# RobustFieldAutonomyLab/DRL_graph_exploration

Hardware: AMD Instinct MI355X
Metric: env-steps/sec (256 parallel envs, ~64-node graphs) (higher is better)
Workload: dtype f64; 1 GPU; configs[1]: 256 envs/GPU, 40x40 map (V=1600), 100 landmarks, belief update at ~59-node graphs (P=37.0 poses, L=22.2 landmarks, M=188 factors) from a device snapshot; envs_per_gpu=256, map_size=40, num_landmarks=100, parallelism=env-sharded x1

## Files before the change

drl_graph_exploration_amd/_lib.py:

```python
import ctypes as C
import os

from .config import DrlgxConfig

_HERE = os.path.dirname(os.path.abspath(__file__))
_PATH = os.environ.get("DRLGX_LIB_DEV", os.path.join(_HERE, "libdrlgx.so"))
_lib = None

N_TIMERS = 8


class DrlgxError(RuntimeError):
    pass


class CsrCache(C.Structure):
    _fields_ = [(n, C.c_void_p) for n in ("deg", "selfw", "ax", "ptr_dst", "end_dst", "ptr_src", "end_src", "nbr_dst", "nbr_src", "wn_dst",
                                          "wn_src")]
    NODE_WORDS = dict(deg=1, selfw=1, ax=8, ptr_dst=1, end_dst=1, ptr_src=1, end_src=1)
    EDGE_WORDS = dict(nbr_dst=1, nbr_src=1, wn_dst=1, wn_src=1)


def lib_path():
    return _PATH


SYMBOLS = [
    "drlgx_create", "drlgx_destroy", "drlgx_set_stream", "drlgx_synchronize", "drlgx_strerror", "drlgx_last_error",
    "drlgx_status_host", "drlgx_status_fetch_host", "drlgx_reset_host", "drlgx_step", "drlgx_utility", "drlgx_uncertainty_em", "drlgx_explored", "drlgx_metrics", "drlgx_cov_array",
    "drlgx_stage_reset_host", "drlgx_stage_set_prior_information_host", "drlgx_stage_set_prior_pose_host", "drlgx_stage_move", "drlgx_stage_measure", "drlgx_stage_add_measurements", "drlgx_stage_optimize",
    "drlgx_stage_update_map", "drlgx_set_planner_parameter", "drlgx_set_fixed_landmarks_host", "drlgx_fm2_update", "drlgx_fm2_update_steps", "drlgx_em_cost", "drlgx_em_cost_steps", "drlgx_set_dubins_leaf_scoring", "drlgx_em_plan_leaves", "drlgx_og_cost", "drlgx_slam_og_cost", "drlgx_set_sampler_parameter", "drlgx_set_sampler_obstacles", "drlgx_set_dubins_library_host", "drlgx_dubins_library", "drlgx_set_dubins_prefilter", "drlgx_em_plan", "drlgx_rrt_plan", "drlgx_step_plan", "drlgx_step_plans", "drlgx_step_plans_traced",
    "drlgx_line_plan", "drlgx_lookahead", "drlgx_lookahead_bounded", "drlgx_graph_capacity", "drlgx_graph", "drlgx_get_counts_host", "drlgx_counts",
    "drlgx_get_poses_host", "drlgx_get_landmarks_host", "drlgx_get_cov_traces_host", "drlgx_vm_shape",
    "drlgx_get_virtual_map_host", "drlgx_get_ground_truth_host", "drlgx_get_adjacency_host", "drlgx_get_factors_host",
    "drlgx_get_landmark_order_host", "drlgx_snapshot", "drlgx_restore", "drlgx_timing_enable",
    "drlgx_timing_read_host", "drlgx_debug_phase_clocks_host", "drlgx_debug_gemm_tile_rows", "drlgx_debug_map_form", "drlgx_debug_map_compact_ok", "drlgx_debug_disc_cells_bound", "drlgx_inc_stats_host", "drlgx_debug_panel_host", "drlgx_gcn_workspace_bytes", "drlgx_gcn_forward", "drlgx_gcn_forward_batched", "drlgx_gcn_backward",
    "drlgx_replay_collate", "drlgx_replay_collate_pair", "drlgx_dqn_targets", "drlgx_dqn_loss_grad", "drlgx_dqn_arena_bytes", "drlgx_dqn_arena_views", "drlgx_dqn_prepare", "drlgx_dqn_forward_backward", "drlgx_replay_cache_csr", "drlgx_gcn_collate_csr", "drlgx_gcn_forward_prebuilt", "drlgx_adam_step", "drlgx_adam_step_scaled", "drlgx_normalise_rewards",
    "drlgx_segment_softmax", "drlgx_segment_softmax_backward", "drlgx_mean_pool", "drlgx_mean_pool_backward",
    "drlgx_ggnn_workspace_bytes", "drlgx_ggnn_forward", "drlgx_ggnn_backward",
    "drlgx_greedy_plans",
    "drlgx_set_env_obstacles", "drlgx_obstacle_flags", "drlgx_follow_plans",
    "drlgx_unet_workspace_bytes", "drlgx_unet_forward", "drlgx_unet_backward", "drlgx_unet_topk", "drlgx_unet_augment_filter", "drlgx_unet_kept_nodes",
]


def lib():
    global _lib
    if _lib is not None:
        return _lib
    import torch
    if not os.path.exists(_PATH):
        raise DrlgxError(
            "libdrlgx.so not found at %s — build it with `python -c 'import __graft_entry__ as g; g.build()'` "
            "(hipcc --offload-arch=gfx950); there is no CPU fallback." % _PATH)
    L = C.CDLL(_PATH)
    vp, ip, dp = C.c_void_p, C.POINTER(C.c_int32), C.POINTER(C.c_double)
    L.drlgx_create.argtypes = [C.POINTER(DrlgxConfig), C.c_int, C.c_int, C.c_int, C.POINTER(vp)]
    L.drlgx_destroy.argtypes = [vp]
    L.drlgx_set_stream.argtypes = [vp, vp]
# ... 54 lines not shown
    L.drlgx_get_counts_host.argtypes = [vp, C.c_int, ip]
    L.drlgx_counts.argtypes = [vp, vp]
    L.drlgx_get_poses_host.argtypes = [vp, C.c_int, dp, dp]
    L.drlgx_get_landmarks_host.argtypes = [vp, C.c_int, ip, dp, dp]
    L.drlgx_get_cov_traces_host.argtypes = [vp, C.c_int, dp, dp]
    L.drlgx_vm_shape.argtypes = [vp, ip, ip]
    L.drlgx_get_virtual_map_host.argtypes = [vp, C.c_int, dp, dp, dp, C.POINTER(C.c_uint8)]
    L.drlgx_get_ground_truth_host.argtypes = [vp, C.c_int, dp, dp]
    L.drlgx_get_adjacency_host.argtypes = [vp, C.c_int, dp, dp]
    L.drlgx_get_factors_host.argtypes = [vp, C.c_int, ip, ip, dp, dp]
    L.drlgx_get_landmark_order_host.argtypes = [vp, ip]
    L.drlgx_snapshot.argtypes = [vp, C.c_int]
    L.drlgx_restore.argtypes = [vp, C.c_int]
    L.drlgx_timing_enable.argtypes = [vp, C.c_int]
    L.drlgx_timing_read_host.argtypes = [vp, dp, C.POINTER(C.c_int64)]
    L.drlgx_debug_phase_clocks_host.argtypes = [vp, C.c_int, C.POINTER(C.c_int64)]
    L.drlgx_debug_gemm_tile_rows.argtypes = [C.c_int, C.c_int, C.c_int, C.c_int]
    L.drlgx_debug_map_form.argtypes = [C.c_int]
    L.drlgx_debug_map_compact_ok.argtypes = [vp, C.c_int]
    L.drlgx_debug_disc_cells_bound.argtypes = [C.c_double]
    L.drlgx_inc_stats_host.argtypes = [vp, C.POINTER(C.c_int64), C.c_int]
    if os.environ.get("DRLGX_LIB_DEV") is None or hasattr(L, "drlgx_debug_panel_host"):
        L.drlgx_debug_panel_host.argtypes = [vp, C.c_int, ip, dp, C.c_size_t]
    L.drlgx_gcn_workspace_bytes.restype = C.c_size_t
    L.drlgx_gcn_workspace_bytes.argtypes = [C.c_int, C.c_int, C.c_int, C.c_int]
    L.drlgx_gcn_forward.argtypes = [vp] + [C.c_int] * 5 + [vp] * 12
    L.drlgx_gcn_backward.argtypes = [vp] + [C.c_int] * 5 + [vp] * 15
    L.drlgx_ggnn_workspace_bytes.restype = C.c_size_t
    L.drlgx_ggnn_workspace_bytes.argtypes = [C.c_int] * 5
    L.drlgx_ggnn_forward.argtypes = [vp] + [C.c_int] * 6 + [vp] * 13 + [C.c_int, vp, vp, C.c_int]
    L.drlgx_ggnn_backward.argtypes = [vp] + [C.c_int] * 6 + [vp] * 17
    L.drlgx_unet_workspace_bytes.restype = C.c_size_t
    L.drlgx_unet_workspace_bytes.argtypes = [C.c_int] * 6 + [C.c_double, C.c_int]
    L.drlgx_unet_forward.argtypes = [vp] + [C.c_int] * 5 + [C.c_double, C.c_int] + [vp] * 3 + [C.POINTER(vp)] + [vp] * 3 + [C.c_size_t, C.c_int, vp, vp,
                                                                                                                       C.c_int]
    L.drlgx_unet_backward.argtypes = [vp] + [C.c_int] * 5 + [C.c_double, C.c_int] + [vp] * 3 + [C.POINTER(vp), vp, vp, C.POINTER(vp), vp, C.c_size_t,
                                                                                                C.c_int, C.c_int]
    L.drlgx_unet_kept_nodes.argtypes = [vp] + [C.c_int] * 4 + [C.c_double, C.c_int, vp, C.c_size_t, C.c_int, C.c_int, C.c_int, vp, C.POINTER(C.c_int)]
    L.drlgx_unet_topk.argtypes = [vp, C.c_int, C.c_int, vp, vp, C.c_double, vp, vp, vp, vp]
    L.drlgx_unet_augment_filter.argtypes = [vp, C.c_int, C.c_int, vp, vp, C.c_int, vp, vp, C.c_int, vp, vp, vp, C.c_int64, vp, vp, vp]
    L.drlgx_replay_collate.argtypes = [vp, C.c_int, vp, vp, C.c_int, vp, C.c_int64, vp, vp, vp, C.c_int64, vp, vp, vp, vp, vp, vp]
    L.drlgx_replay_collate_pair.argtypes = [vp, C.c_int, vp, vp, C.c_int, vp, C.c_int64, vp, vp, vp, C.c_int64, vp, vp, vp, vp, vp, vp, vp]
    L.drlgx_gcn_forward_batched.argtypes = [vp] + [C.c_int] * 5 + [vp] * 12 + [C.c_int, vp, vp, C.c_int]
    L.drlgx_dqn_targets.argtypes = [vp, C.c_int, vp, vp, vp, C.c_double, C.c_int64, vp, vp]
    L.drlgx_dqn_loss_grad.argtypes = [vp, C.c_int, vp, vp, vp, C.c_double, vp, vp]
    i64 = C.c_int64
# ... 41 lines not shown
```

drl_graph_exploration_amd/csrc/drlgx_dev.h:

```cpp
#pragma once
#include <hip/hip_runtime.h>
#include <stdint.h>

#include "../../include/drlgx.h"
#include "map_carve.h"

#define DRLGX_MT_N 624
#define DRLGX_MT_STRIDE 626
#define DRLGX_CNT_STRIDE 8
#define DRLGX_RED_STRIDE 8
#define DRLGX_PRIOR_STRIDE 16

enum { C_P = 0, C_L = 1, C_M = 2, C_STEP = 3, C_ISAM = 4, C_NEWP = 5, C_NEWL = 6, C_FLAG = 7 };
enum { R_UTR = 0, R_KNOWN = 1, R_EXPL = 2, R_UDET = 3, R_UWTR = 4, R_DIST = 5, R_OBS = 6, R_LATCH = 7 };

struct DrlgxState {
  drlgx_config cfg;
  int n_envs, n_inst, n_roll;
  int P_max, L_max, M_max, LG, V, Vu, rows, cols, A_max;
  int win;
  int disc_cells;
  int count_explored;
  double lo_free, lo_occ, lo_min, lo_max, occ_thresh;
  int bbox_noop;
// ... 559 lines not shown
size_t drlgx_simlog_entry_bytes(const DrlgxState &S);
void drlgx_launch_presim(const DrlgxState &S, hipStream_t st, LaunchSel sel, const double *odom, int odom_stride, int n_measure, int a_end,
                         unsigned char *simlog, size_t simlog_roll, int simlog_act);
void drlgx_launch_sim(const DrlgxState &S, hipStream_t st, LaunchSel sel, const double *odom, int odom_stride,
                      int n_measure);
void drlgx_launch_sim_obs(const DrlgxState &S, hipStream_t st, LaunchSel sel, const double *odom, int odom_stride);
void drlgx_launch_slam(const DrlgxState &S, hipStream_t st, LaunchSel sel, int p_bound);
size_t drlgx_map_lds_bytes(const DrlgxState &S, int *chunk_out, int pcap = 0);
bool drlgx_step_fusable(const DrlgxState &S, int p_bound);
bool drlgx_step_arrow_fusable(const DrlgxState &S);
void drlgx_launch_step_arrow(const DrlgxState &S, hipStream_t st, LaunchSel sel, const double *odom, int odom_stride, int n_measure);
void drlgx_launch_step(const DrlgxState &S, hipStream_t st, LaunchSel sel, const double *odom, int odom_stride, int n_measure);
void drlgx_launch_step_loop(const DrlgxState &S, hipStream_t st, LaunchSel sel, const double *odom, int odom_stride, int n_measure, int a_end);
void drlgx_launch_step_arrow_loop(const DrlgxState &S, hipStream_t st, LaunchSel sel, const double *odom, int odom_stride, int n_measure, int a_end);
void drlgx_launch_map(const DrlgxState &S, hipStream_t st, LaunchSel sel, int rebuild);
bool drlgx_map_two_per_cu(const DrlgxState &S, int p_bound);
bool drlgx_map_compact_ok(const DrlgxState &S, int p_bound);
void drlgx_launch_copy(const DrlgxField *fields_dev, int n_fields, hipStream_t st, int n, const int32_t *src,
                       const int32_t *dst, int src_off, int dst_off, int skip_mask,
                       const int *cnt = nullptr,
                       const DrlgxState *panel = nullptr,
                       int only_cls = -1,
                       int panel_mode = 1);
void drlgx_launch_rebase(const DrlgxState &S, hipStream_t st, int base0, int n);
inline size_t drlgx_fetch_head_bytes(int n_envs) { return ((size_t)(n_envs + 1) * sizeof(int) + 15) & ~(size_t)15; }
void drlgx_launch_fetch_pack(const DrlgxState &S, hipStream_t st, const void *src, size_t bytes, void *out);
void drlgx_launch_fix_rollouts(const DrlgxState &S, hipStream_t st, int n_cand, const int32_t *cand_env, int roll0);
void drlgx_launch_rewards(const DrlgxState &S, hipStream_t st, int n_cand, const int32_t *cand_env, int roll0,
                          double *rewards);
void drlgx_launch_utility(const DrlgxState &S, hipStream_t st, const double *dist, double *out, int mode);
void drlgx_launch_fm2_prior(const DrlgxState &S, hipStream_t st, const int32_t *env_ids, int n_env, double *sig, size_t sig_stride,
                            int n_max);
size_t drlgx_fm2_scratch_doubles(const DrlgxState &S, int nm_max);
void drlgx_launch_fm2_check(const DrlgxState &S, hipStream_t st, int n_cand, const int32_t *cand_env, const double *actions,
                            const int32_t *n_actions, const uint8_t *core, int nm_max, int *flag);
void drlgx_launch_fm2_update(const DrlgxState &S, hipStream_t st, int c0, int nc, const int32_t *cand_env, const int32_t *env_slot,
                             const double *actions, const int32_t *n_actions, const uint8_t *core, const double *sig, size_t sig_stride,
                             double *scratch, size_t scratch_stride, int *iscratch, int nm_max, double *cov_out, int out_stride,
                             int32_t *n_out, double *lm_out = nullptr, int lm_stride = 0);
void drlgx_launch_fm2_prior_ordered(const DrlgxState &S, hipStream_t st, double *sig, size_t sig_stride, int n_max);
size_t drlgx_em_lds_bytes(const DrlgxState &S);
void drlgx_launch_em_cost(const DrlgxState &S, hipStream_t st, int nc, const int32_t *cand_env, const double *actions,
                          const int32_t *n_actions, const uint8_t *core, const double *distance, const double *cov, int cov_stride,
                          int algorithm, double *unc_out, double *cost_out, double *info_out);
size_t drlgx_og_lds_bytes(const DrlgxState &S);
void drlgx_launch_og_check(const DrlgxState &S, hipStream_t st, int n_cand, const int32_t *cand_env, const int32_t *n_actions, int *flag);
// ... 61 lines not shown
```

drl_graph_exploration_amd/csrc/drlgx_engine.cpp:

```cpp
#include <hip/hip_runtime.h>

#include <algorithm>
#include <chrono>
#include <cmath>
#include <cstdio>
#include <cstring>
#include <functional>
#include <string>
#include <unordered_map>
#include <cstdlib>
#include <vector>

#include "drlgx_dev.h"
#include "drlgx_fields.h"

#define HIPCHK(e, call)                                                                       \
  do {                                                                                        \
    hipError_t _r = (call);                                                                   \
    if (_r != hipSuccess) {                                                                   \
      (e)->last_error = std::string(#call) + ": " + hipGetErrorString(_r);                    \
      return DRLGX_E_HIP;                                                                     \
    }                                                                                         \
  } while (0)

struct TimedSpan {
  hipEvent_t a, b;
  int id;
};

struct drlgx_engine {
  DrlgxState S{};
  int device = 0;
  hipStream_t own_stream = nullptr, stream = nullptr;
  std::vector<void *> allocs;
  DrlgxState *state_dev = nullptr;
  unsigned char state_shadow[sizeof(DrlgxState)];
  std::vector<DrlgxField> fields;
  DrlgxField *fields_dev = nullptr;
  std::vector<int> lm_order;
  int32_t *stage_i32 = nullptr;
  uint32_t *stage_u32 = nullptr;
  double *stage_f64 = nullptr;
  uint8_t *stage_mask = nullptr;
  int *graph_gi = nullptr;
  int graph_gi_stride = 0;
  bool timing = false;
  std::vector<int> pbound;
  bool by_capacity = false;
  std::vector<std::vector<int>> snap_pbound;
  bool per_stage = false;
  std::vector<TimedSpan> spans;
  std::vector<hipEvent_t> free_events;
  double t_ms[DRLGX_N_TIMERS] = {0};
  int64_t t_n[DRLGX_N_TIMERS] = {0};
  std::string last_error;
  double *fixed_lm_dev = nullptr;
  unsigned char *simlog_dev = nullptr;
  bool la_presim = true;
  bool spin_sync = true;
  hipEvent_t sync_event = nullptr;
  unsigned char *fetch_dev = nullptr, *fetch_host = nullptr;
// ... 14 lines not shown
  int *tree_link = nullptr, *tree_leaf = nullptr, *tree_meta = nullptr;
  int32_t *tree_cand_env = nullptr, *tree_cand_n = nullptr;
  size_t tree_nodes_cap = 0, tree_sel_cap = 0, tree_cand_cap = 0;
  double sampler_max_nodes = 0.5, sampler_safe_distance = 0.0;
  int sampler_dubins = 0;
  int sampler_obstacles = 0;
  int env_obstacles = 0;
  double *follow_act = nullptr;
  int dubins_leaf_scoring = 0;
  uint8_t *tree_cand_core = nullptr;
  double *tree_cand_dist = nullptr;
  size_t tree_cand_steps_cap = 0, tree_cand_last = 0;
  bool tree_cand_last_steps = false;
  DrlgxDubins dubins = {};
  double *dub_end_x = nullptr, *dub_end_y = nullptr, *dub_v = nullptr, *dub_w = nullptr, *tree_pose = nullptr;
  int *dub_steps = nullptr;
  size_t dub_cap = 0, tree_pose_cap = 0;
  double dub_reach = 0.0;
  int dub_prefilter = 1;
  std::vector<double> dub_end_h, dub_v_h, dub_w_h;
  std::vector<int> dub_steps_h;
  int owed_slot = -1;
  bool restore_eager = false;
};

#define DRLGX_ENTER_OWING(e)                    \
  do {                                          \
    if (e) {                                    \
      (void)hipSetDevice((e)->device);          \
      state_sync(e);                            \
    }                                           \
  } while (0)
#define DRLGX_ENTER(e)                          \
  do {                                          \
    DRLGX_ENTER_OWING(e);                       \
    if (e) settle(e);                           \
  } while (0)

struct drlgx_engine;
static void state_sync(drlgx_engine *e);
static void settle(drlgx_engine *e);

namespace {

template <typename T>
int dev_alloc(drlgx_engine *e, T **out, size_t count) {
// ... 86 lines not shown
  }
  const int LG = std::max(cfg->num_landmarks, 1);
  if (drlgx_sim_launch_lds(DRLGX_SIM_RESET, LG) > kSimLdsLimit || drlgx_sim_launch_lds(DRLGX_SIM_STEP, LG) > kSimLdsLimit ||
      drlgx_sim_launch_lds(DRLGX_SIM_STAGE, LG) > kSimLdsLimit ||
      (n_rollouts > 0 && drlgx_sim_launch_lds(DRLGX_SIM_PRESIM, LG, 1) > kSimLdsLimit)) {
    g_create_error = "num_landmarks too large for the LDS of the simulator kernels (k_reset / k_sim_step / k_presim)";
    return DRLGX_E_INVALID;
  }
  return DRLGX_OK;
}

static bool env_flag(const char *name, bool dflt) {
  const char *v = getenv(name);
  if (!v) return dflt;
  return dflt ? v[0] != '0' : v[0] == '1';
}

static void read_env_switches(drlgx_engine *e) {
  e->by_capacity = env_flag("DRLGX_VARIANT_BY_CAPACITY", false);
  e->spin_sync = env_flag("DRLGX_SYNC_SPIN", true);
  e->la_presim = env_flag("DRLGX_LOOKAHEAD_PRESIM", true);
  e->la_loop = env_flag("DRLGX_LOOKAHEAD_LOOP", true);
  e->restore_eager = env_flag("DRLGX_RESTORE_EAGER", false);
}

static double p2l(double p) { return std::log(p / (1.0 - p)); }
static double l2p(double l) { return std::exp(l) / (1.0 + std::exp(l)); }

static int disc_cells_bound(double r) {
  const int n = 32;
  const double h = 0.5 / n, rr = r + h * 0.70710678118654752440 + 1e-9;
  const int k = (int)std::ceil(rr) + 1;
  int best = 0;
  for (int a = 0; a < n; ++a)
    for (int b = 0; b < n; ++b) {
      const double u = (a + 0.5) * h, v = (b + 0.5) * h;
      int cnt = 0;
      for (int i = -k; i <= k; ++i)
        for (int j = -k; j <= k; ++j)
          if ((i - u) * (i - u) + (j - v) * (j - v) <= rr * rr) ++cnt;
      best = std::max(best, cnt);
    }
  return best;
}

static int set_map_constants(drlgx_engine *e) {
// ... 192 lines not shown
    while (e->allocs.size() > n_before) {
      hipFree(e->allocs.back());
      e->allocs.pop_back();
    }
    S.jc = nullptr;
    S.jd = nullptr;
    S.jc_meta = nullptr;
    S.inc_stats = nullptr;
    e->last_error.clear();
    fprintf(stderr, "drlgx: covariance panels (%.1f GB) not allocated (budget %.1f GB): every belief update is a full solve\n", gb, max_gb);
  }
  return DRLGX_OK;
}

static int alloc_staging(drlgx_engine *e) {
  DrlgxState &S = e->S;
  const int n_envs = S.n_envs;
  TRY(dev_alloc(e, &S.status, 1));
  std::stable_sort(e->fields.begin(), e->fields.end(), [](const DrlgxField &a, const DrlgxField &b) {
    return (a.pad > 0 ? (size_t)a.pad : a.stride) > (b.pad > 0 ? (size_t)b.pad : b.stride);
  });
  TRY(dev_alloc(e, &e->fields_dev, e->fields.size()));
  HIPCHK(e, hipMemcpyAsync(e->fields_dev, e->fields.data(), e->fields.size() * sizeof(DrlgxField), hipMemcpyHostToDevice, e->stream));
  TRY(dev_alloc(e, &e->stage_i32, (size_t)n_envs));
  TRY(dev_alloc(e, &e->stage_u32, (size_t)n_envs));
  TRY(dev_alloc(e, &e->stage_f64, (size_t)n_envs * 3));
  TRY(dev_alloc(e, &e->stage_mask, (size_t)n_envs));
  e->graph_gi_stride = 4 * S.L_max + 8;
  TRY(dev_alloc(e, &e->graph_gi, (size_t)n_envs * e->graph_gi_stride));
  unsigned char *raw = nullptr;
  TRY(dev_alloc(e, &raw, sizeof(DrlgxState)));
  e->state_dev = reinterpret_cast<DrlgxState *>(raw);
  S.self_dev = e->state_dev;
  return DRLGX_OK;
}

static int build_engine(drlgx_engine *e) {
  DrlgxState &S = e->S;
  const drlgx_config *cfg = &S.cfg;
  if (cfg->max_snapshots < 0 || cfg->max_snapshots > 16) return DRLGX_E_INVALID;
  S.n_inst = 2 * S.n_envs + S.n_roll + cfg->max_snapshots * S.n_envs;
  e->pbound.assign(S.n_envs, cfg->max_poses);
  e->snap_pbound.assign(cfg->max_snapshots > 0 ? cfg->max_snapshots : 0, std::vector<int>(S.n_envs, cfg->max_poses));
  read_env_switches(e);
  hipDeviceProp_t prop;
  if (hipGetDeviceProperties(&prop, e->device) == hipSuccess && prop.multiProcessorCount > 0) e->n_cu = prop.multiProcessorCount;
// ... 145 lines not shown
  hipError_t r = hipEventRecord(e->sync_event, e->stream);
  if (r != hipSuccess) return r;
  const auto t0 = std::chrono::steady_clock::now();
  for (int polls = 0; (r = hipEventQuery(e->sync_event)) == hipErrorNotReady; ++polls) {
    if ((polls & 63) == 63 && std::chrono::steady_clock::now() - t0 > std::chrono::microseconds(5000)) return hipStreamSynchronize(e->stream);
  }
  return r;
}

static int status_fetch(drlgx_engine *e, const void *src_dev, size_t bytes, void *dst_host) {
  const size_t head = drlgx_fetch_head_bytes(e->S.n_envs), total = head + ((bytes + 15) & ~(size_t)15);
  if (total > e->fetch_cap) {
    HIPCHK(e, hipStreamSynchronize(e->stream));
    if (e->fetch_dev) (void)hipFree(e->fetch_dev);
    if (e->fetch_host) (void)hipHostFree(e->fetch_host);
    e->fetch_dev = e->fetch_host = nullptr;
    e->fetch_cap = 0;
    const size_t cap = std::max<size_t>(2 * total, 1 << 16);
    HIPCHK(e, hipMalloc(reinterpret_cast<void **>(&e->fetch_dev), cap));
    HIPCHK(e, hipHostMalloc(reinterpret_cast<void **>(&e->fetch_host), cap, hipHostMallocDefault));
    e->fetch_cap = cap;
  }
  drlgx_launch_fetch_pack(e->S, e->stream, src_dev, bytes, e->fetch_dev);
  HIPCHK(e, hipMemcpyAsync(e->fetch_host, e->fetch_dev, head + bytes, hipMemcpyDeviceToHost, e->stream));
  HIPCHK(e, stream_wait(e));
  const int32_t *h = reinterpret_cast<const int32_t *>(e->fetch_host);
  for (int i = 0; i < e->S.n_envs; ++i) e->pbound[i] = std::min(std::max((int)h[1 + i], 1), e->S.P_max);
  if (bytes) std::memcpy(dst_host, e->fetch_host + head, bytes);
  return h[0];
}

int drlgx_status_host(drlgx_engine *e) {
  DRLGX_ENTER_OWING(e);
  if (!e) return DRLGX_E_INVALID;
  return status_fetch(e, nullptr, 0, nullptr);
}

int drlgx_status_fetch_host(drlgx_engine *e, const void *src_dev, size_t bytes, void *dst_host) {
  DRLGX_ENTER_OWING(e);
  if (!e || (bytes > 0 && (!src_dev || !dst_host))) return DRLGX_E_INVALID;
  return status_fetch(e, src_dev, bytes, dst_host);
}

int drlgx_reset_host(drlgx_engine *e, int n, const int32_t *env_ids, const uint32_t *seeds, const double *start) {
  DRLGX_ENTER(e);
  if (!e || n <= 0 || n > e->S.n_envs || !env_ids || !seeds || !start) return DRLGX_E_INVALID;
// ... 1077 lines not shown
      features[a] = pt[mp[m]];
      features[b] = lt[ml[m]];
    }
  }
  return DRLGX_OK;
}

int drlgx_get_landmark_order_host(const drlgx_engine *e, int32_t *order) {
  if (!e || !order) return DRLGX_E_INVALID;
  for (int i = 0; i < e->S.cfg.num_landmarks; ++i) order[i] = e->lm_order[i];
  return DRLGX_OK;
}

int drlgx_snapshot(drlgx_engine *e, int slot) {
  DRLGX_ENTER(e);
  if (!e || slot < 0 || slot >= e->S.cfg.max_snapshots) return DRLGX_E_INVALID;
  const DrlgxState &S = e->S;
  ScopedTimer t(e, 3);
  drlgx_launch_copy(e->fields_dev, (int)e->fields.size(), e->stream, S.n_envs, nullptr, nullptr, 0, snapshot_base(e, slot), 0, e->S.cnt, &S);
  e->snap_pbound[slot] = e->pbound;
  return check_launch(e);
}

int drlgx_restore(drlgx_engine *e, int slot) {
  DRLGX_ENTER_OWING(e);
  if (!e || slot < 0 || slot >= e->S.cfg.max_snapshots) return DRLGX_E_INVALID;
  const DrlgxState &S = e->S;
  ScopedTimer t(e, 3);
  drlgx_launch_copy(e->fields_dev, (int)e->fields.size(), e->stream, S.n_envs, nullptr, nullptr, snapshot_base(e, slot), 0,
                    e->restore_eager ? 0 : 1, e->S.cnt, &S, -1, e->restore_eager ? 1 : 2);
  e->owed_slot = e->restore_eager ? -1 : slot;
  e->pbound = e->snap_pbound[slot];
  return check_launch(e);
}

int drlgx_debug_phase_clocks_host(drlgx_engine *e, int arm, int64_t out[64]) {
  DRLGX_ENTER(e);
  if (!e) return DRLGX_E_INVALID;
  HIPCHK(e, hipStreamSynchronize(e->stream));
  e->S.prof_block = (arm >> 8) & 0xffff;
  if (out && e->S.prof)
    HIPCHK(e, hipMemcpy(out, e->S.prof + ((arm & 4) ? 0 : ((arm & 2) ? 64 : 0)), ((arm & 4) ? 1024 : 64) * sizeof(long long), hipMemcpyDeviceToHost));
  if (arm && !e->S.prof) {
    long long *p = nullptr;
    int r = dev_alloc(e, &p, 1024);
    if (r) return r;
    HIPCHK(e, hipStreamSynchronize(e->stream));
    e->S.prof = p;
  } else if (!arm) {
    e->S.prof = nullptr;
  }
  return DRLGX_OK;
}
// ... 15 lines not shown
int drlgx_debug_panel_host(drlgx_engine *e, int inst, int32_t meta[4], double *panel, size_t panel_cap) {
  DRLGX_ENTER(e);
  if (!INST_OK(e, inst) || !meta) return DRLGX_E_INVALID;
  const DrlgxState &S = e->S;
  meta[0] = meta[1] = meta[2] = meta[3] = 0;
  if (!S.jc) return DRLGX_OK;
  int r = fetch(e, meta, S.jc_meta + (size_t)inst * 4, 4 * sizeof(int32_t));
  if (r) return r;
  HIPCHK(e, hipStreamSynchronize(e->stream));
  if (!panel || meta[0] != 1) return DRLGX_OK;
  const int P = meta[1], L = meta[2];
  if (P < 0 || P > S.P_max || L < 0 || L > S.L_max) return DRLGX_E_INVALID;
  const size_t cols = 3 + 2 * (size_t)L, rows = 3 * (size_t)P + 2 * (size_t)L;
  if (rows * cols > panel_cap) return DRLGX_E_INVALID;
  const double *src = S.jc + (size_t)inst * S.jc_stride;
  if (P > 0) HIPCHK(e, hipMemcpy2DAsync(panel, cols * 8, src, (size_t)S.jc_ld * 8, cols * 8, 3 * (size_t)P, hipMemcpyDeviceToHost, e->stream));
  if (L > 0)
    HIPCHK(e, hipMemcpy2DAsync(panel + 3 * (size_t)P * cols, cols * 8, src + 3 * (size_t)S.P_max * S.jc_ld, (size_t)S.jc_ld * 8, cols * 8,
                               2 * (size_t)L, hipMemcpyDeviceToHost, e->stream));
  HIPCHK(e, hipStreamSynchronize(e->stream));
  return DRLGX_OK;
}

int drlgx_timing_enable(drlgx_engine *e, int on) {
  DRLGX_ENTER_OWING(e);
  if (!e) return DRLGX_E_INVALID;
  e->timing = on != 0;
  e->per_stage = on == 2;
  return DRLGX_OK;
}

int drlgx_timing_read_host(drlgx_engine *e, double ms[DRLGX_N_TIMERS], int64_t launches[DRLGX_N_TIMERS]) {
  DRLGX_ENTER_OWING(e);
  if (!e) return DRLGX_E_INVALID;
  HIPCHK(e, hipStreamSynchronize(e->stream));
  for (auto &sp : e->spans) {
    float t = 0;
    if (hipEventElapsedTime(&t, sp.a, sp.b) == hipSuccess && sp.id >= 0 && sp.id < DRLGX_N_TIMERS) {
      e->t_ms[sp.id] += t;
      e->t_n[sp.id] += 1;
    }
    e->free_events.push_back(sp.a);
    e->free_events.push_back(sp.b);
  }
  e->spans.clear();
  for (int i = 0; i < DRLGX_N_TIMERS; ++i) {
// ... 10 lines not shown
```

drl_graph_exploration_amd/csrc/drlgx_fields.h:

```cpp
#pragma once
#include <stddef.h>
struct DrlgxField {
  char *base;
  size_t stride;
  int cls;
  int unit;
  int unit_bytes;
  int pad;
};
```

drl_graph_exploration_amd/csrc/k_misc.hip:

```cpp
#include "drlgx_dev.h"
#include "drlgx_fields.h"

namespace {

constexpr int kCopySplit = 8;
__device__ __forceinline__ void copy_panel_part(const DrlgxState &S, int s, int d, int part, int mode) {
  const int *ms = S.jc_meta + (size_t)s * 4;
  int *md = S.jc_meta + (size_t)d * 4;
  const int valid = ms[0] & ~kPanelInSrc, P = ms[1], L = ms[2], M = ms[3];
  if (threadIdx.x == 0 && part == 0) {
    if (mode != 3) {
      md[0] = (mode == 2 && valid == 1) ? (valid | kPanelInSrc) : valid; md[1] = P; md[2] = L; md[3] = M;
    } else if (valid == 1) {
      md[0] = valid;
    }
  }
  if (valid != 1) return;
  if (mode != 2) drlgx_copy_panel_body<256>(S.jc, S.jc_stride, S.jc_ld, S.P_max, s, d, P, L, part, kCopySplit, threadIdx.x);
  if (part == 0 && mode != 3)
    for (int e = threadIdx.x; e < 6 * P; e += 256) S.jd[(size_t)d * S.P_max * 6 + e] = S.jd[(size_t)s * S.P_max * 6 + e];
}

__global__ __launch_bounds__(256) void k_copy_instances(const DrlgxField *fields, int n_fields, const int32_t *src,
                                                        const int32_t *dst, int src_off, int dst_off, int skip_mask, int only_cls,
                                                        const int *cnt, DrlgxState S, int panel) {
  const int i = blockIdx.y;
  const int f = blockIdx.x;
  const int s = (src ? src[i] : i) + src_off, d = (dst ? dst[i] : i) + dst_off;
  if (f >= n_fields) {
    if (panel) copy_panel_part(S, s, d, f - n_fields, panel);
    return;
  }
  if ((fields[f].cls & skip_mask) || (only_cls >= 0 && fields[f].cls != only_cls)) return;
  const size_t stride = fields[f].stride;
  const char *sb = fields[f].base + (size_t)s * stride;
  char *db = fields[f].base + (size_t)d * stride;
  size_t live = fields[f].pad > 0 ? (size_t)fields[f].pad : stride;
  if (fields[f].unit && cnt) {
    const int *c = cnt + (size_t)s * DRLGX_CNT_STRIDE;
    const int k = fields[f].unit == 1 ? c[C_P] : fields[f].unit == 2 ? c[C_L] : c[C_M];
    const size_t b = ((size_t)(k > 0 ? k : 0) * (size_t)fields[f].unit_bytes + 15) & ~(size_t)15;
    live = b < stride ? b : stride;
  }
  if ((stride & 15) == 0) {
    const uint4 *sp = reinterpret_cast<const uint4 *>(sb);
    uint4 *dp = reinterpret_cast<uint4 *>(db);
    const size_t nq = live / 16;
    size_t k = threadIdx.x;
    for (; k + 256 < nq; k += 512) {
      const uint4 v0 = sp[k], v1 = sp[k + 256];
      dp[k] = v0; dp[k + 256] = v1;
    }
    if (k < nq) dp[k] = sp[k];
  } else {
    const uint32_t *sp = reinterpret_cast<const uint32_t *>(sb);
    uint32_t *dp = reinterpret_cast<uint32_t *>(db);
    const size_t nw = (live < stride ? live : stride) / 4;
    for (size_t k = threadIdx.x; k < nw; k += 256) dp[k] = sp[k];
  }
}

__global__ __launch_bounds__(256) void k_fetch_pack(const int *status, const int *cnt, int n_envs, int head, const unsigned char *src,
                                                    size_t bytes, unsigned char *out) {
  const size_t t = (size_t)blockIdx.x * 256 + threadIdx.x, nt = (size_t)gridDim.x * 256;
  int *h = reinterpret_cast<int *>(out);
  for (size_t i = t; i < (size_t)n_envs + 1; i += nt) h[i] = i == 0 ? status[0] : cnt[(i - 1) * DRLGX_CNT_STRIDE + C_P];
  unsigned char *o = out + head;
  if (((reinterpret_cast<uintptr_t>(src) | bytes) & 15) == 0) {
    const uint4 *s4 = reinterpret_cast<const uint4 *>(src);
    uint4 *o4 = reinterpret_cast<uint4 *>(o);
    for (size_t i = t; i < bytes / 16; i += nt) o4[i] = s4[i];
  } else {
    for (size_t i = t; i < bytes; i += nt) o[i] = src[i];
  }
}

__global__ __launch_bounds__(64) void k_rebase(DrlgxState S, int base0, int n) {
  const int inst = base0 + blockIdx.x;
  int *cnt = S.cnt + (size_t)inst * DRLGX_CNT_STRIDE;
  const int P = cnt[C_P], L = cnt[C_L];
  for (int i = threadIdx.x; i < P; i += 64) {
// ... 318 lines not shown
  hipLaunchKernelGGL(k_follow_select, dim3(S.n_envs), dim3(64), 0, st, S, plan, n_actions, result, active, steps, fallback[0], fallback[1],
                     fallback[2], act, n_exec, stop);
}
void drlgx_launch_follow_record(const DrlgxState &S, hipStream_t st, double sigma0, int a, const double *act, int32_t *n_exec, int obstacles,
                                double done_explored, int max_steps, double *trace, int32_t *done, int32_t *stop) {
  hipLaunchKernelGGL(k_follow_record, dim3(S.n_envs), dim3(256), 0, st, S, sigma0, a, act, n_exec, obstacles, done_explored, max_steps, trace,
                     done, stop);
}
void drlgx_launch_obstacle_flags(const DrlgxState &S, hipStream_t st, uint8_t *out) {
  hipLaunchKernelGGL(k_obstacle_flags, dim3((S.n_envs + 127) / 128), dim3(128), 0, st, S, out);
}
void drlgx_launch_cov_array(const DrlgxState &S, hipStream_t st, double *length, double *angle) {
  hipLaunchKernelGGL(k_cov_array, dim3((S.V + 255) / 256, S.n_envs), dim3(256), 0, st, S, length, angle);
}
void drlgx_launch_copy(const DrlgxField *fields_dev, int n_fields, hipStream_t st, int n, const int32_t *src,
                       const int32_t *dst, int src_off, int dst_off, int skip_mask, const int *cnt, const DrlgxState *panel,
                       int only_cls, int panel_mode) {
  if (n <= 0) return;
  const bool with_panel = panel && panel->jc;
  const dim3 cgrid(n_fields + (with_panel ? kCopySplit : 0), n);
  hipLaunchKernelGGL(k_copy_instances, cgrid, dim3(256), 0, st, fields_dev, n_fields, src, dst,
                     src_off, dst_off, skip_mask, only_cls, cnt, with_panel ? *panel : DrlgxState{}, with_panel ? panel_mode : 0);
}
void drlgx_launch_fetch_pack(const DrlgxState &S, hipStream_t st, const void *src, size_t bytes, void *out) {
  const size_t head = drlgx_fetch_head_bytes(S.n_envs);
  const int blocks = (int)std::min<size_t>(256, (head + bytes + 4095) / 4096);
  hipLaunchKernelGGL(k_fetch_pack, dim3(std::max(blocks, 1)), dim3(256), 0, st, S.status, S.cnt, S.n_envs, (int)head,
                     reinterpret_cast<const unsigned char *>(src), bytes, reinterpret_cast<unsigned char *>(out));
}
void drlgx_launch_rebase(const DrlgxState &S, hipStream_t st, int base0, int n) {
  hipLaunchKernelGGL(k_rebase, dim3(n), dim3(64), 0, st, S, base0, n);
}
void drlgx_launch_fix_rollouts(const DrlgxState &S, hipStream_t st, int n_cand, const int32_t *cand_env, int roll0) {
  hipLaunchKernelGGL(k_fix_rollouts, dim3(n_cand), dim3(64), 0, st, S, cand_env, roll0);
}
void drlgx_launch_rewards(const DrlgxState &S, hipStream_t st, int n_cand, const int32_t *cand_env, int roll0,
                          double *rewards) {
  hipLaunchKernelGGL(k_rewards, dim3((n_cand + 127) / 128), dim3(128), 0, st, S, n_cand, cand_env, roll0, rewards);
}
void drlgx_launch_utility(const DrlgxState &S, hipStream_t st, const double *dist, double *out, int mode) {
  hipLaunchKernelGGL(k_utility, dim3((S.n_envs + 127) / 128), dim3(128), 0, st, S, dist, out, mode);
}
void drlgx_launch_line_plan(const DrlgxState &S, hipStream_t st, int n_cand, const int32_t *cand_env, const double *goal,
                            double *actions, int32_t *n_actions) {
  hipLaunchKernelGGL(k_line_plan, dim3((n_cand + 127) / 128), dim3(128), 0, st, S, n_cand, cand_env, goal, actions,
                     n_actions);
// ... 14 lines not shown
```

drl_graph_exploration_amd/engine.py:

```python
import ctypes as C
import math

import numpy as np
import torch

from . import _lib
from .config import DrlgxConfig, start_pose


def _p(t):
    return C.c_void_p(t.data_ptr()) if t is not None else None


_NP_OF = {torch.float32: np.float32, torch.float64: np.float64, torch.int32: np.int32, torch.int64: np.int64, torch.uint8: np.uint8,
          torch.bool: np.bool_, torch.int16: np.int16, torch.int8: np.int8}


class Engine(object):
    def __init__(self, cfg, n_envs, n_rollouts=0, device=0):
        if not isinstance(cfg, DrlgxConfig):
            raise TypeError("cfg must be a DrlgxConfig")
        if not torch.cuda.is_available():
            raise _lib.DrlgxError("no HIP device visible: the drlgx engine has no CPU fallback")
        self.L = _lib.lib()
# ... 465 lines not shown
    def snapshot(self, slot=0):
        self.use_torch_stream()
        self._chk(self.L.drlgx_snapshot(self.h, slot))

    def restore(self, slot=0):
        self.use_torch_stream()
        self._chk(self.L.drlgx_restore(self.h, slot))

    def inc_stats(self, reset=False):
        out = (C.c_int64 * 2)()
        self._chk(self.L.drlgx_inc_stats_host(self.h, out, 1 if reset else 0))
        return int(out[0]), int(out[1])

    def panel(self, inst):
        meta = np.zeros(4, dtype=np.int32)
        ipt, dpt = C.POINTER(C.c_int32), C.POINTER(C.c_double)
        self._chk(self.L.drlgx_debug_panel_host(self.h, inst, meta.ctypes.data_as(ipt), None, 0))
        if meta[0] != 1:
            return meta, None
        body = np.zeros((3 * meta[1] + 2 * meta[2], 3 + 2 * meta[2]))
        self._chk(self.L.drlgx_debug_panel_host(self.h, inst, meta.ctypes.data_as(ipt), body.ctypes.data_as(dpt), body.size))
        return meta, body

    def snapshot_instance(self, slot, env):
        return 2 * self.n_envs + self.n_rollouts + slot * self.n_envs + env

    def timing_enable(self, on=True):
        self._chk(self.L.drlgx_timing_enable(self.h, int(on)))

    def timing_read(self):
        ms = (C.c_double * _lib.N_TIMERS)()
        n = (C.c_int64 * _lib.N_TIMERS)()
        self._chk(self.L.drlgx_timing_read_host(self.h, ms, n))
        names = ["sim", "slam", "map", "copy", "graph", "step", "t6", "t7"]
        return {names[i]: (ms[i], n[i]) for i in range(_lib.N_TIMERS)}

    def counts(self, inst):
        out = (C.c_int32 * 5)()
        self._chk(self.L.drlgx_get_counts_host(self.h, inst, out))
        return dict(poses=out[0], landmarks=out[1], factors=out[2], step=out[3], isam_count=out[4])

    def counts_dev(self):
        self.use_torch_stream()
        out = torch.empty(self.n_envs, 5, dtype=torch.int32, device=self.device)
        self._chk(self.L.drlgx_counts(self.h, _p(out)))
        return out
# ... 70 lines not shown
```

include/drlgx.h:

```cpp
#ifndef DRLGX_H
#define DRLGX_H

#include <stddef.h>
#include <stdint.h>

#ifdef __cplusplus
extern "C" {
#endif

#define DRLGX_OK 0
#define DRLGX_E_INVALID (-1)
#define DRLGX_E_NODEVICE (-2)
#define DRLGX_E_CAPACITY (-3)
#define DRLGX_E_HIP (-4)
#define DRLGX_E_NUMERIC (-5)

#define DRLGX_ALG_EM_AOPT 0
#define DRLGX_ALG_EM_DOPT 1

typedef struct drlgx_config {
  double bearing_noise, range_noise, min_bearing, max_bearing, min_range, max_range;
  double translation_noise, rotation_noise;
  double env_min_x, env_max_x, env_min_y, env_max_y, safe_distance;
  double map_min_x, map_max_x, map_min_y, map_max_y;
// ... 125 lines not shown
int drlgx_get_adjacency_host(drlgx_engine *e, int inst, double *adjacency, double *features);
int drlgx_get_factors_host(drlgx_engine *e, int inst, int32_t *pose, int32_t *key, double *bearing, double *range);
int drlgx_get_landmark_order_host(const drlgx_engine *e, int32_t *order);

int drlgx_snapshot(drlgx_engine *e, int slot);
int drlgx_restore(drlgx_engine *e, int slot);

#define DRLGX_N_TIMERS 8
int drlgx_timing_enable(drlgx_engine *e, int on);
int drlgx_timing_read_host(drlgx_engine *e, double ms[DRLGX_N_TIMERS], int64_t launches[DRLGX_N_TIMERS]);

int drlgx_debug_phase_clocks_host(drlgx_engine *e, int arm, int64_t *out );

int drlgx_debug_gemm_tile_rows(int m, int n, int k_slices, int transpose_a);

int drlgx_debug_map_form(int form);

int drlgx_debug_map_compact_ok(const drlgx_engine *e, int p_bound);

int drlgx_debug_disc_cells_bound(double radius_cells);

int drlgx_inc_stats_host(drlgx_engine *e, int64_t out[2], int reset);
int drlgx_debug_panel_host(drlgx_engine *e, int inst, int32_t meta[4], double *panel, size_t panel_cap);


size_t drlgx_gcn_workspace_bytes(int n_nodes, int n_edges, int hidden, int out_dim);
int drlgx_gcn_forward(void *hip_stream, int n_nodes, int n_edges, int in_dim, int hidden, int out_dim,
                      const float *x, const int64_t *edge_index, const float *edge_attr, const float *W1,
                      const float *b1, const float *W2, const float *b2, const float *Wf, const float *bf,
                      const float *dropout_mask , float *out ,
                      void *ws_dev);
int drlgx_gcn_forward_batched(void *hip_stream, int n_nodes, int n_edges, int in_dim, int hidden, int out_dim,
                              const float *x, const int64_t *edge_index, const float *edge_attr, const float *W1,
                              const float *b1, const float *W2, const float *b2, const float *Wf, const float *bf,
                              const float *dropout_mask, float *out, void *ws_dev, int n_graphs,
                              const int32_t *node_off, const int32_t *edge_off, int max_edges_per_graph);
int drlgx_gcn_backward(void *hip_stream, int n_nodes, int n_edges, int in_dim, int hidden, int out_dim,
                       const float *x, const int64_t *edge_index, const float *edge_attr, const float *W1,
                       const float *W2, const float *Wf, const float *dropout_mask, const float *d_out,
                       float *dW1, float *db1, float *dW2, float *db2, float *dWf, float *dbf, void *ws_dev);


size_t drlgx_ggnn_workspace_bytes(int n_nodes, int n_edges, int hidden, int n_layers, int out_dim);
int drlgx_ggnn_forward(void *hip_stream, int n_nodes, int n_edges, int in_dim, int hidden, int n_layers, int out_dim,
                       const float *x, const int64_t *edge_index, const float *edge_attr,
                       const float *weight , const float *w_ih , const float *w_hh,
// ... 101 lines not shown
```

Measured before the change: 4.217 million env-steps/sec.

## Add compact flattened restore kernel copying live field bytes per env

Adds a dedicated restore kernel that launches one block per env. The block builds a prefix table of live items across all non-class-1 fields, including the joint panel, and copies them as a single flattened stream. 16-byte fields use vector loads and word-strided fields use 4-byte loads, with several loads kept in flight per thread. This replaces the generic per-field copy kernel on the restore path to cut launch imbalance and idle threads on small live regions. The trade-off is a binary search over the table for each item and a 32-entry table limit; the old path remains as the fallback.

```diff
diff --git a/drl_graph_exploration_amd/_lib.py b/drl_graph_exploration_amd/_lib.py
--- a/drl_graph_exploration_amd/_lib.py
+++ b/drl_graph_exploration_amd/_lib.py
@@ -34,7 +34,7 @@
     "drlgx_get_poses_host", "drlgx_get_landmarks_host", "drlgx_get_cov_traces_host", "drlgx_vm_shape",
     "drlgx_get_virtual_map_host", "drlgx_get_ground_truth_host", "drlgx_get_adjacency_host", "drlgx_get_factors_host",
     "drlgx_get_landmark_order_host", "drlgx_snapshot", "drlgx_restore", "drlgx_timing_enable",
-    "drlgx_timing_read_host", "drlgx_debug_phase_clocks_host", "drlgx_debug_gemm_tile_rows", "drlgx_debug_map_form", "drlgx_debug_map_compact_ok", "drlgx_debug_disc_cells_bound", "drlgx_inc_stats_host", "drlgx_debug_panel_host", "drlgx_gcn_workspace_bytes", "drlgx_gcn_forward", "drlgx_gcn_forward_batched", "drlgx_gcn_backward",
+    "drlgx_timing_read_host", "drlgx_debug_phase_clocks_host", "drlgx_debug_gemm_tile_rows", "drlgx_debug_map_form", "drlgx_debug_map_compact_ok", "drlgx_debug_disc_cells_bound", "drlgx_inc_stats_host", "drlgx_debug_panel_host", "drlgx_debug_restore_table_host", "drlgx_debug_field_live_bytes", "drlgx_gcn_workspace_bytes", "drlgx_gcn_forward", "drlgx_gcn_forward_batched", "drlgx_gcn_backward",
     "drlgx_replay_collate", "drlgx_replay_collate_pair", "drlgx_dqn_targets", "drlgx_dqn_loss_grad", "drlgx_dqn_arena_bytes", "drlgx_dqn_arena_views", "drlgx_dqn_prepare", "drlgx_dqn_forward_backward", "drlgx_replay_cache_csr", "drlgx_gcn_collate_csr", "drlgx_gcn_forward_prebuilt", "drlgx_adam_step", "drlgx_adam_step_scaled", "drlgx_normalise_rewards",
     "drlgx_segment_softmax", "drlgx_segment_softmax_backward", "drlgx_mean_pool", "drlgx_mean_pool_backward",
     "drlgx_ggnn_workspace_bytes", "drlgx_ggnn_forward", "drlgx_ggnn_backward",
@@ -135,6 +135,10 @@
     L.drlgx_inc_stats_host.argtypes = [vp, C.POINTER(C.c_int64), C.c_int]
     if os.environ.get("DRLGX_LIB_DEV") is None or hasattr(L, "drlgx_debug_panel_host"):
         L.drlgx_debug_panel_host.argtypes = [vp, C.c_int, ip, dp, C.c_size_t]
+    if os.environ.get("DRLGX_LIB_DEV") is None or hasattr(L, "drlgx_debug_restore_table_host"):
+        L.drlgx_debug_restore_table_host.argtypes = [vp, ip, C.POINTER(C.c_int64), C.c_int]
+        L.drlgx_debug_field_live_bytes.restype = C.c_int64
+        L.drlgx_debug_field_live_bytes.argtypes = [C.c_int64, C.c_int, C.c_int, C.c_int, C.c_int]
     L.drlgx_gcn_workspace_bytes.restype = C.c_size_t
     L.drlgx_gcn_workspace_bytes.argtypes = [C.c_int, C.c_int, C.c_int, C.c_int]
     L.drlgx_gcn_forward.argtypes = [vp] + [C.c_int] * 5 + [vp] * 12
diff --git a/drl_graph_exploration_amd/csrc/drlgx_dev.h b/drl_graph_exploration_amd/csrc/drlgx_dev.h
--- a/drl_graph_exploration_amd/csrc/drlgx_dev.h
+++ b/drl_graph_exploration_amd/csrc/drlgx_dev.h
@@ -605,6 +605,9 @@
                        const DrlgxState *panel = nullptr,
                        int only_cls = -1,
                        int panel_mode = 1);
+void drlgx_launch_restore_compact(const DrlgxField *tab_dev, int n_tab, int n16, hipStream_t st, int n, int src_off, const int *cnt,
+                                  int *jc_meta);
+int drlgx_restore_items_per_trip();
 void drlgx_launch_rebase(const DrlgxState &S, hipStream_t st, int base0, int n);
 inline size_t drlgx_fetch_head_bytes(int n_envs) { return ((size_t)(n_envs + 1) * sizeof(int) + 15) & ~(size_t)15; }
 void drlgx_launch_fetch_pack(const DrlgxState &S, hipStream_t st, const void *src, size_t bytes, void *out);
diff --git a/drl_graph_exploration_amd/csrc/drlgx_engine.cpp b/drl_graph_exploration_amd/csrc/drlgx_engine.cpp
--- a/drl_graph_exploration_amd/csrc/drlgx_engine.cpp
+++ b/drl_graph_exploration_amd/csrc/drlgx_engine.cpp
@@ -37,6 +37,9 @@
   unsigned char state_shadow[sizeof(DrlgxState)];
   std::vector<DrlgxField> fields;
   DrlgxField *fields_dev = nullptr;
+  std::vector<DrlgxField> restore_tab;
+  DrlgxField *restore_tab_dev = nullptr;
+  int restore_n16 = 0;
   std::vector<int> lm_order;
   int32_t *stage_i32 = nullptr;
   uint32_t *stage_u32 = nullptr;
@@ -97,6 +100,7 @@
   std::vector<int> dub_steps_h;
   int owed_slot = -1;
   bool restore_eager = false;
+  bool restore_compact = true;
 };
 
 #define DRLGX_ENTER_OWING(e)                    \
@@ -229,6 +233,7 @@
   e->la_presim = env_flag("DRLGX_LOOKAHEAD_PRESIM", true);
   e->la_loop = env_flag("DRLGX_LOOKAHEAD_LOOP", true);
   e->restore_eager = env_flag("DRLGX_RESTORE_EAGER", false);
+  e->restore_compact = env_flag("DRLGX_RESTORE_COMPACT", true);
 }
 
 static double p2l(double p) { return std::log(p / (1.0 - p)); }
@@ -467,6 +472,9 @@
   });
   TRY(dev_alloc(e, &e->fields_dev, e->fields.size()));
   HIPCHK(e, hipMemcpyAsync(e->fields_dev, e->fields.data(), e->fields.size() * sizeof(DrlgxField), hipMemcpyHostToDevice, e->stream));
+  e->restore_tab = drlgx_restore_table(e->fields, S.jd, S.P_max, &e->restore_n16);
+  TRY(dev_alloc(e, &e->restore_tab_dev, e->restore_tab.size()));
+  HIPCHK(e, hipMemcpyAsync(e->restore_tab_dev, e->restore_tab.data(), e->restore_tab.size() * sizeof(DrlgxField), hipMemcpyHostToDevice, e->stream));
   TRY(dev_alloc(e, &e->stage_i32, (size_t)n_envs));
   TRY(dev_alloc(e, &e->stage_u32, (size_t)n_envs));
   TRY(dev_alloc(e, &e->stage_f64, (size_t)n_envs * 3));
@@ -658,6 +666,7 @@
     e->fetch_cap = cap;
   }
   drlgx_launch_fetch_pack(e->S, e->stream, src_dev, bytes, e->fetch_dev);
+  if (int r = check_launch(e)) return r;
   HIPCHK(e, hipMemcpyAsync(e->fetch_host, e->fetch_dev, head + bytes, hipMemcpyDeviceToHost, e->stream));
   HIPCHK(e, stream_wait(e));
   const int32_t *h = reinterpret_cast<const int32_t *>(e->fetch_host);
@@ -1781,13 +1790,21 @@
   return check_launch(e);
 }
 
+static bool restore_is_compact(const drlgx_engine *e) {
+  return e->restore_compact && !e->restore_eager && (int)e->restore_tab.size() <= kRestoreMaxEntries;
+}
+
 int drlgx_restore(drlgx_engine *e, int slot) {
   DRLGX_ENTER_OWING(e);
   if (!e || slot < 0 || slot >= e->S.cfg.max_snapshots) return DRLGX_E_INVALID;
   const DrlgxState &S = e->S;
   ScopedTimer t(e, 3);
-  drlgx_launch_copy(e->fields_dev, (int)e->fields.size(), e->stream, S.n_envs, nullptr, nullptr, snapshot_base(e, slot), 0,
-                    e->restore_eager ? 0 : 1, e->S.cnt, &S, -1, e->restore_eager ? 1 : 2);
+  if (restore_is_compact(e))
+    drlgx_launch_restore_compact(e->restore_tab_dev, (int)e->restore_tab.size(), e->restore_n16, e->stream, S.n_envs, snapshot_base(e, slot),
+                                 S.cnt, S.jc ? S.jc_meta : nullptr);
+  else
+    drlgx_launch_copy(e->fields_dev, (int)e->fields.size(), e->stream, S.n_envs, nullptr, nullptr, snapshot_base(e, slot), 0,
+                      e->restore_eager ? 0 : 1, e->S.cnt, &S, -1, e->restore_eager ? 1 : 2);
   e->owed_slot = e->restore_eager ? -1 : slot;
   e->pbound = e->snap_pbound[slot];
   return check_launch(e);
@@ -1849,6 +1866,28 @@
   return DRLGX_OK;
 }
 
+int drlgx_debug_restore_table_host(const drlgx_engine *e, int32_t info[4], int64_t *rows, int rows_cap) {
+  if (!e || !info) return DRLGX_E_INVALID;
+  const int n = (int)e->restore_tab.size();
+  info[0] = n;
+  info[1] = e->restore_n16;
+  info[2] = restore_is_compact(e) ? 1 : 0;
+  info[3] = drlgx_restore_items_per_trip();
+  for (int k = 0; rows && k < n && k < rows_cap; ++k) {
+    const DrlgxField &f = e->restore_tab[k];
+    rows[4 * k] = (int64_t)f.stride;
+    rows[4 * k + 1] = f.unit;
+    rows[4 * k + 2] = f.unit_bytes;
+    rows[4 * k + 3] = f.pad;
+  }
+  return DRLGX_OK;
+}
+
+int64_t drlgx_debug_field_live_bytes(int64_t stride, int unit, int unit_bytes, int pad, int count) {
+  if (stride < 0 || unit < 0 || unit_bytes < 0) return -1;
+  return (int64_t)drlgx_field_live_bytes((size_t)stride, unit, unit_bytes, pad, count);
+}
+
 int drlgx_timing_enable(drlgx_engine *e, int on) {
   DRLGX_ENTER_OWING(e);
   if (!e) return DRLGX_E_INVALID;
diff --git a/drl_graph_exploration_amd/csrc/drlgx_fields.h b/drl_graph_exploration_amd/csrc/drlgx_fields.h
--- a/drl_graph_exploration_amd/csrc/drlgx_fields.h
+++ b/drl_graph_exploration_amd/csrc/drlgx_fields.h
@@ -1,5 +1,6 @@
 #pragma once
 #include <stddef.h>
+#include <vector>
 struct DrlgxField {
   char *base;
   size_t stride;
@@ -8,3 +9,23 @@
   int unit_bytes;
   int pad;
 };
+
+__host__ __device__ inline size_t drlgx_field_live_bytes(size_t stride, int unit, int unit_bytes, int pad, int count) {
+  if (!unit) return pad > 0 ? (size_t)pad : stride;
+  const size_t b = ((size_t)(count > 0 ? count : 0) * (size_t)unit_bytes + 15) & ~(size_t)15;
+  return b < stride ? b : stride;
+}
+__host__ __device__ inline bool drlgx_field_by_words(size_t stride) { return (stride & 15) != 0; }
+__host__ __device__ inline size_t drlgx_field_items(size_t stride, size_t live) { return drlgx_field_by_words(stride) ? live / 4 : live / 16; }
+
+constexpr int kRestoreMaxEntries = 32;
+inline std::vector<DrlgxField> drlgx_restore_table(const std::vector<DrlgxField> &fields, const double *jd, int P_max, int *n16) {
+  std::vector<DrlgxField> tab;
+  for (const DrlgxField &f : fields)
+    if (f.cls != 1 && !drlgx_field_by_words(f.stride)) tab.push_back(f);
+  if (jd) tab.push_back(DrlgxField{reinterpret_cast<char *>(const_cast<double *>(jd)), (size_t)P_max * 6 * sizeof(double), 0, 4, 6 * (int)sizeof(double), 0});
+  *n16 = (int)tab.size();
+  for (const DrlgxField &f : fields)
+    if (f.cls != 1 && drlgx_field_by_words(f.stride)) tab.push_back(f);
+  return tab;
+}
diff --git a/drl_graph_exploration_amd/csrc/k_misc.hip b/drl_graph_exploration_amd/csrc/k_misc.hip
--- a/drl_graph_exploration_amd/csrc/k_misc.hip
+++ b/drl_graph_exploration_amd/csrc/k_misc.hip
@@ -35,14 +35,14 @@
   const size_t stride = fields[f].stride;
   const char *sb = fields[f].base + (size_t)s * stride;
   char *db = fields[f].base + (size_t)d * stride;
-  size_t live = fields[f].pad > 0 ? (size_t)fields[f].pad : stride;
-  if (fields[f].unit && cnt) {
+  const int unit = cnt ? fields[f].unit : 0;
+  int count = 0;
+  if (unit) {
     const int *c = cnt + (size_t)s * DRLGX_CNT_STRIDE;
-    const int k = fields[f].unit == 1 ? c[C_P] : fields[f].unit == 2 ? c[C_L] : c[C_M];
-    const size_t b = ((size_t)(k > 0 ? k : 0) * (size_t)fields[f].unit_bytes + 15) & ~(size_t)15;
-    live = b < stride ? b : stride;
-  }
-  if ((stride & 15) == 0) {
+    count = unit == 1 ? c[C_P] : unit == 2 ? c[C_L] : c[C_M];
+  }
+  const size_t live = drlgx_field_live_bytes(stride, unit, fields[f].unit_bytes, fields[f].pad, count);
+  if (!drlgx_field_by_words(stride)) {
     const uint4 *sp = reinterpret_cast<const uint4 *>(sb);
     uint4 *dp = reinterpret_cast<uint4 *>(db);
     const size_t nq = live / 16;
@@ -57,6 +57,96 @@
     uint32_t *dp = reinterpret_cast<uint32_t *>(db);
     const size_t nw = (live < stride ? live : stride) / 4;
     for (size_t k = threadIdx.x; k < nw; k += 256) dp[k] = sp[k];
+  }
+}
+
+constexpr int kRestoreDepth = 4, kRestoreWordDepth = 2;
+#ifndef DRLGX_RESTORE_THREADS
+#define DRLGX_RESTORE_THREADS 512
+#endif
+constexpr int kRestoreThreads = DRLGX_RESTORE_THREADS;
+
+typedef unsigned int restore_q __attribute__((ext_vector_type(4)));
+typedef __attribute__((address_space(1))) restore_q restore_gq;
+typedef __attribute__((address_space(1))) uint32_t restore_gw;
+
+__device__ __forceinline__ int restore_entry_of(const unsigned *pre, unsigned i) {
+  int k = 0;
+#pragma unroll
+  for (int step = kRestoreMaxEntries / 2; step; step >>= 1)
+    if (pre[k + step] <= i) k += step;
+  return k;
+}
+
+template <int T>
+__global__ __launch_bounds__(T) void k_restore_compact(const DrlgxField *__restrict__ tab, int n_tab, int n16, int src_off,
+                                                       const int *__restrict__ cnt, int *jc_meta) {
+  __shared__ unsigned pre[kRestoreMaxEntries + 1];
+  __shared__ uintptr_t src_of[kRestoreMaxEntries], dst_of[kRestoreMaxEntries];
+  const int d = blockIdx.x, s = d + src_off, tid = threadIdx.x;
+  if (tid < 64) {
+    const DrlgxField f = tab[tid < n_tab ? tid : n_tab - 1];
+    const int *c = cnt + (size_t)s * DRLGX_CNT_STRIDE;
+    const int *ms = jc_meta ? jc_meta + (size_t)s * 4 : c;
+    static_assert(DRLGX_CNT_STRIDE == 8, "the lanes read the counts' row by tid & 7");
+    const int cv = c[tid & 7], hv = ms[tid & 3];
+    const int cP = __shfl(cv, C_P), cL = __shfl(cv, C_L), cM = __shfl(cv, C_M);
+    const int valid = jc_meta ? __shfl(hv, 0) & ~kPanelInSrc : 0, mP = __shfl(hv, 1), mL = __shfl(hv, 2), mM = __shfl(hv, 3);
+    unsigned items = 0;
+    if (tid < n_tab) {
+      const int count = f.unit == 1 ? cP : f.unit == 2 ? cL : f.unit == 3 ? cM : valid == 1 ? mP : 0;
+      items = (unsigned)drlgx_field_items(f.stride, drlgx_field_live_bytes(f.stride, f.unit, f.unit_bytes, f.pad, count));
+      src_of[tid] = reinterpret_cast<uintptr_t>(f.base + (size_t)s * f.stride);
+      dst_of[tid] = reinterpret_cast<uintptr_t>(f.base + (size_t)d * f.stride);
+    }
+    unsigned incl = items;
+#pragma unroll
+    for (int o = 1; o < 64; o <<= 1) {
+      const unsigned up = __shfl_up(incl, o);
+      if (tid >= o) incl += up;
+    }
+    if (tid <= kRestoreMaxEntries) pre[tid] = incl - items;
+    if (tid == 0 && jc_meta) {
+      int *md = jc_meta + (size_t)d * 4;
+      md[0] = valid == 1 ? (valid | kPanelInSrc) : valid; md[1] = mP; md[2] = mL; md[3] = mM;
+    }
+  }
+  __syncthreads();
+  const unsigned N16 = pre[n16], N = pre[kRestoreMaxEntries];
+  for (unsigned a = tid, b = N16 + tid; a < N16 || b < N; a += T * kRestoreDepth, b += T * kRestoreWordDepth) {
+    int kv[kRestoreDepth], kw[kRestoreWordDepth];
+#pragma unroll
+    for (int j = 0; j < kRestoreDepth; ++j) kv[j] = restore_entry_of(pre, a + j * T);
+#pragma unroll
+    for (int j = 0; j < kRestoreWordDepth; ++j) kw[j] = restore_entry_of(pre, b + j * T);
+    restore_q v[kRestoreDepth];
+    restore_gq *vp[kRestoreDepth];
+    uint32_t w[kRestoreWordDepth];
+    restore_gw *wp[kRestoreWordDepth];
+#pragma unroll
+    for (int j = 0; j < kRestoreDepth; ++j) {
+      const unsigned i = a + j * T;
+      const size_t off = i - pre[kv[j]];
+      const restore_gq *sp = (const restore_gq *)src_of[kv[j]] + off;
+      vp[j] = (restore_gq *)dst_of[kv[j]] + off;
+      v[j] = restore_q{0, 0, 0, 0};
+      if (i < N16) v[j] = *sp;
+    }
+#pragma unroll
+    for (int j = 0; j < kRestoreWordDepth; ++j) {
+      const unsigned i = b + j * T;
+      const size_t off = i - pre[kw[j]];
+      const restore_gw *sp = (const restore_gw *)src_of[kw[j]] + off;
+      wp[j] = (restore_gw *)dst_of[kw[j]] + off;
+      w[j] = 0;
+      if (i < N) w[j] = *sp;
+    }
+#pragma unroll
+    for (int j = 0; j < kRestoreDepth; ++j)
+      if (a + j * T < N16) *vp[j] = v[j];
+#pragma unroll
+    for (int j = 0; j < kRestoreWordDepth; ++j)
+      if (b + j * T < N) *wp[j] = w[j];
   }
 }
 
@@ -421,6 +511,12 @@
   hipLaunchKernelGGL(k_copy_instances, cgrid, dim3(256), 0, st, fields_dev, n_fields, src, dst,
                      src_off, dst_off, skip_mask, only_cls, cnt, with_panel ? *panel : DrlgxState{}, with_panel ? panel_mode : 0);
 }
+void drlgx_launch_restore_compact(const DrlgxField *tab_dev, int n_tab, int n16, hipStream_t st, int n, int src_off, const int *cnt,
+                                  int *jc_meta) {
+  if (n <= 0) return;
+  hipLaunchKernelGGL(k_restore_compact<kRestoreThreads>, dim3(n), dim3(kRestoreThreads), 0, st, tab_dev, n_tab, n16, src_off, cnt, jc_meta);
+}
+int drlgx_restore_items_per_trip() { return kRestoreThreads * kRestoreDepth; }
 void drlgx_launch_fetch_pack(const DrlgxState &S, hipStream_t st, const void *src, size_t bytes, void *out) {
   const size_t head = drlgx_fetch_head_bytes(S.n_envs);
   const int blocks = (int)std::min<size_t>(256, (head + bytes + 4095) / 4096);
diff --git a/drl_graph_exploration_amd/engine.py b/drl_graph_exploration_amd/engine.py
--- a/drl_graph_exploration_amd/engine.py
+++ b/drl_graph_exploration_amd/engine.py
@@ -511,6 +511,14 @@
         self._chk(self.L.drlgx_debug_panel_host(self.h, inst, meta.ctypes.data_as(ipt), body.ctypes.data_as(dpt), body.size))
         return meta, body
 
+    def restore_table(self):
+        info = np.zeros(4, dtype=np.int32)
+        ipt, lpt = C.POINTER(C.c_int32), C.POINTER(C.c_int64)
+        self._chk(self.L.drlgx_debug_restore_table_host(self.h, info.ctypes.data_as(ipt), None, 0))
+        rows = np.zeros((int(info[0]), 4), dtype=np.int64)
+        self._chk(self.L.drlgx_debug_restore_table_host(self.h, info.ctypes.data_as(ipt), rows.ctypes.data_as(lpt), rows.shape[0]))
+        return dict(entries=int(info[0]), entries_16=int(info[1]), in_use=bool(info[2]), items_per_trip=int(info[3])), rows
+
     def snapshot_instance(self, slot, env):
         return 2 * self.n_envs + self.n_rollouts + slot * self.n_envs + env
 
diff --git a/include/drlgx.h b/include/drlgx.h
--- a/include/drlgx.h
+++ b/include/drlgx.h
@@ -171,6 +171,9 @@
 
 int drlgx_inc_stats_host(drlgx_engine *e, int64_t out[2], int reset);
 int drlgx_debug_panel_host(drlgx_engine *e, int inst, int32_t meta[4], double *panel, size_t panel_cap);
+
+int drlgx_debug_restore_table_host(const drlgx_engine *e, int32_t info[4], int64_t *rows, int rows_cap);
+int64_t drlgx_debug_field_live_bytes(int64_t stride, int unit, int unit_bytes, int pad, int count);
 
 
 size_t drlgx_gcn_workspace_bytes(int n_nodes, int n_edges, int hidden, int out_dim);
```

Measured after the change: 4.417 million env-steps/sec (median of 6 runs). 1.05x the previous value.
